# neonnnnn/nimfm

Measured on AMD Instinct MI355X. Metric: SGD training samples/sec/epoch, higher is better.
Workload: dtype f64

## Files before the change

include/nimfm_hip.h:

```cpp
#ifndef NIMFM_HIP_H
#define NIMFM_HIP_H
#include <stdint.h>

#ifdef __cplusplus
extern "C" {
#endif

#define NFM_OK 0
#define NFM_ERR_INVALID (-1)
#define NFM_ERR_HIP (-2)
#define NFM_ERR_NOT_FITTED (-3)
#define NFM_ERR_NOMEM (-4)
#define NFM_ERR_UNSUPPORTED (-5)

typedef struct nfm_ctx nfm_ctx;
typedef struct nfm_dataset nfm_dataset;
typedef struct nfm_model nfm_model;
typedef struct nfm_opt nfm_opt;

enum { NFM_TASK_REGRESSION = 0, NFM_TASK_CLASSIFICATION = 1 };
enum { NFM_KIND_FM = 0, NFM_KIND_FFM = 1, NFM_KIND_CFM = 2  };
enum { NFM_LOWER_EXPLICIT = 0, NFM_LOWER_AUGMENT = 1, NFM_LOWER_NONE = 2 };
enum { NFM_LOSS_SQUARED = 0, NFM_LOSS_SQUARED_HINGE = 1, NFM_LOSS_LOGISTIC = 2, NFM_LOSS_HUBER = 3 };
enum { NFM_SCHED_CONSTANT = 0, NFM_SCHED_OPTIMAL = 1, NFM_SCHED_INVSCALING = 2, NFM_SCHED_PEGASOS = 3 };
// ... 57 lines not shown
enum { NFM_LAYOUT_CSR = 0, NFM_LAYOUT_CSC = 1 };
int32_t nfm_dataset_create_csc(nfm_ctx* ctx, int64_t n_samples, int64_t n_features,
                               const int64_t* indptr , const int64_t* indices ,
                               const double* data , const double* y , nfm_dataset** out);
int32_t nfm_dataset_create_csc_device(nfm_ctx* ctx, int64_t n_samples, int64_t n_features, int64_t nnz,
                                      const int64_t* indptr_dev, const int32_t* indices_dev, const double* data_dev,
                                      const double* y_dev, nfm_dataset** out);
int32_t nfm_dataset_to_csc(nfm_dataset* ds, nfm_dataset** out);
int32_t nfm_dataset_to_csr(nfm_dataset* ds, nfm_dataset** out);
int32_t nfm_dataset_layout(const nfm_dataset* ds, int32_t* layout);
int32_t nfm_dataset_get_csc(nfm_dataset* ds, int64_t* indptr , int64_t* indices , double* data );
int32_t nfm_dataset_load_user_item_lines(nfm_ctx* ctx, const char* path, int32_t short_lines, nfm_dataset** out);
int32_t nfm_dataset_parse_user_item_lines(nfm_ctx* ctx, const char* text, int64_t len, int32_t short_lines, nfm_dataset** out);
int32_t nfm_dataset_shape(const nfm_dataset* ds, int64_t* n_samples, int64_t* n_features,
                          int64_t* nnz, int64_t* n_fields);
int32_t nfm_dataset_ingest_stats(const nfm_dataset* ds, int64_t* bytes, double* upload_ms,
                                 double* parse_ms);
int32_t nfm_dataset_get_targets(nfm_dataset* ds, double* y );
int32_t nfm_dataset_get_csr(nfm_dataset* ds, int64_t* indptr , int64_t* indices ,
                            double* data , int64_t* fields );
int32_t nfm_dataset_set_targets(nfm_dataset* ds, const double* y);
int32_t nfm_dataset_destroy(nfm_dataset* ds);

typedef struct nfm_model_cfg {
  int32_t kind;
  int32_t task;
  int32_t degree;
  int32_t n_components;
  int32_t fit_lower;
  int32_t fit_intercept;
// ... 129 lines not shown
```

nimfm_amd/_capi.py:

```python
import atexit
import ctypes as C
import os
import subprocess

_HERE = os.path.dirname(os.path.abspath(__file__))
LIB_PATH = os.environ.get("NIMFM_HIP_LIB") or os.path.join(_HERE, "lib", "libnimfm_hip.so")
CSRC = os.path.join(_HERE, "csrc")

NFM_OK = 0
ERR_INVALID, ERR_HIP, ERR_NOT_FITTED, ERR_NOMEM, ERR_UNSUPPORTED = -1, -2, -3, -4, -5

TASK = {"regression": 0, "r": 0, "classification": 1, "c": 1}
KIND_FM, KIND_FFM, KIND_CFM = 0, 1, 2
LOWER = {"explicit": 0, "augment": 1, "none": 2}
LOSS = {"squared": 0, "squared_hinge": 1, "logistic": 2, "huber": 3}
SCHED = {"constant": 0, "optimal": 1, "invscaling": 2, "pegasos": 3}
MODE = {"sequential": 0, "minibatch": 1}
REG = {"l1": 0, "l21": 1, "squaredl12": 2, "squaredl21": 3, "omegati": 4, "omegacs": 5}
NORM = {"l1": 0, "l2": 1, "linfty": 2}
LAYOUT = {"csr": 0, "csc": 1}

SYMBOLS = [
    "nfm_last_error", "nfm_version", "nfm_device_count",
    "nfm_ctx_create", "nfm_ctx_destroy", "nfm_ctx_synchronize",
# ... 11 lines not shown
    "nfm_dp_unique_id", "nfm_dp_create", "nfm_dp_create_local", "nfm_dp_info", "nfm_dp_destroy", "nfm_opt_set_dp", "nfm_opt_set_dp_combine", "nfm_opt_set_touch_cap", "nfm_opt_set_ada_cross",
    "nfm_opt_set_shuffle", "nfm_opt_get_perm", "nfm_opt_announce_perm",
    "nfm_stream_open", "nfm_stream_shape", "nfm_stream_load_rows", "nfm_stream_prefetch_rows", "nfm_stream_close",
    "nfm_cd_create", "nfm_cd_begin_fit", "nfm_cd_schedule", "nfm_pcd_create", "nfm_pbcd_create",
    "nfm_pgd_create", "nfm_pgd_begin_fit", "nfm_pgd_last_iter",
    "nfm_katyusha_create", "nfm_katyusha_begin_fit", "nfm_katyusha_snapshot",
    "nfm_cfm_create", "nfm_cfm_set_params", "nfm_cfm_get_params",
    "nfm_hazan_create", "nfm_hazan_begin_fit", "nfm_hazan_iter", "nfm_rng_rand_uniform",
    "nfm_gcd_create", "nfm_gcd_begin_fit", "nfm_gcd_outer_begin", "nfm_gcd_inner", "nfm_gcd_outer_end",
    "nfm_psgd_create", "nfm_psgd_begin_fit", "nfm_psgd_finalize",
    "nfm_dataset_select_rows", "nfm_dataset_slice_rows", "nfm_dataset_vstack", "nfm_dataset_hstack", "nfm_dataset_normalize",
    "nfm_dataset_load_user_item", "nfm_dataset_parse_user_item", "nfm_rng_shuffle_forward",
    "nfm_dataset_dump_svmlight", "nfm_dataset_dump_ffm", "nfm_dataset_format_text", "nfm_dump_stats", "nfm_format_f64",
    "nfm_dataset_create_csc", "nfm_dataset_create_csc_device", "nfm_dataset_to_csc", "nfm_dataset_to_csr", "nfm_dataset_layout", "nfm_dataset_get_csc",
    "nfm_dataset_load_user_item_lines", "nfm_dataset_parse_user_item_lines",
]


class ModelCfg(C.Structure):
    _fields_ = [("kind", C.c_int32), ("task", C.c_int32), ("degree", C.c_int32), ("n_components", C.c_int32),
                ("fit_lower", C.c_int32), ("fit_intercept", C.c_int32), ("fit_linear", C.c_int32),
                ("reserved", C.c_int32), ("n_features", C.c_int64), ("n_fields", C.c_int64)]


class SGDCfg(C.Structure):
    _fields_ = [("eta0", C.c_double), ("alpha0", C.c_double), ("alpha", C.c_double), ("beta", C.c_double),
                ("power", C.c_double), ("loss_param", C.c_double), ("loss", C.c_int32), ("scheduling", C.c_int32),
                ("mode", C.c_int32), ("reserved", C.c_int32), ("batch", C.c_int64)]


# ... 156 lines not shown
        "nfm_dataset_hstack": [vp, i64, pp],
        "nfm_dataset_normalize": [vp, i32, i32, pp],
        "nfm_dataset_load_user_item": [vp, C.c_char_p, pp],
        "nfm_dataset_parse_user_item": [vp, C.c_char_p, i64, pp],
        "nfm_rng_shuffle_forward": [vp, vp, i64],
        "nfm_dataset_dump_svmlight": [vp, C.c_char_p, vp, i32, i64],
        "nfm_dataset_dump_ffm": [vp, C.c_char_p, vp, i32, i64],
        "nfm_dataset_format_text": [vp, vp, i32, i64, vp, i64, C.POINTER(i64)],
        "nfm_dump_stats": [C.POINTER(i64), C.POINTER(i64), C.POINTER(dbl), C.POINTER(dbl), C.POINTER(dbl)],
        "nfm_format_f64": [vp, vp, i64, i64, vp, i64, C.POINTER(i64)],
        "nfm_dataset_create_csc": [vp, i64, i64, vp, vp, vp, vp, pp],
        "nfm_dataset_create_csc_device": [vp, i64, i64, i64, vp, vp, vp, vp, pp],
        "nfm_dataset_to_csc": [vp, pp],
        "nfm_dataset_to_csr": [vp, pp],
        "nfm_dataset_layout": [vp, C.POINTER(i32)],
        "nfm_dataset_get_csc": [vp, vp, vp, vp],
        "nfm_dataset_load_user_item_lines": [vp, C.c_char_p, i32, pp],
        "nfm_dataset_parse_user_item_lines": [vp, C.c_char_p, i64, i32, pp],
    }
    for name, args in sig.items():
        fn = getattr(L, name)
        fn.argtypes = args
        fn.restype = C.c_int32
    _lib = L
    return L


def check(rc):
    if rc == NFM_OK:
        return
# ... 7 lines not shown
```

nimfm_amd/csrc/api.hip:

```cpp
#include <fcntl.h>
#include <math.h>
#include <string.h>
#include <unistd.h>

#include <algorithm>
#include <atomic>
#include <condition_variable>
#include <map>
#include <mutex>
#include <memory>
#include <string>
#include <thread>
#include <vector>

#include "cd.h"
#include "cfm.h"
#include "dataset_csc.h"
#include "dataset_ops.h"
#include "dataset_text.h"
#include "gcd.h"
#include "psgd_seq.h"
#include "dp.h"
#include "ingest.h"
#include "mb.h"
#include "katyusha.h"
#include "pgd.h"

using namespace nfm;

struct nfm_dataset {
  nfm_ctx* ctx = nullptr;
  CsrView v{};
  DevBuf indptr, indices, data, fields, y;
  bool has_y = false;
  int max_row = 0;
  int64_t repeats = 0, repeat_row = -1;
  int64_t ingest_bytes = 0;
  double ingest_upload_ms = 0.0, ingest_parse_ms = 0.0;
  uint64_t uid = 0, serial = 0;
  uint64_t y_gen = 0;
  CscIndex csc;
  int layout = NFM_LAYOUT_CSR;
  DevBuf c_indptr, c_indices, c_data;
  CsrView cv{};
};
static int refuse_csc(const nfm_dataset* ds, const char* what) {
  NFM_CHECK(ds->layout != NFM_LAYOUT_CSC, NFM_ERR_UNSUPPORTED,
            "%s takes a row-major dataset, not a CSCDataset: convert it with toCSRDataset (nfm_dataset_to_csr)", what);
  return NFM_OK;
}
static uint64_t next_dataset_uid() {
// ... 347 lines not shown
    NFM_HIP_CHECK(hipStreamSynchronize(st));
  }
  if (y) {
    NFM_TRY(ds->y.alloc(sizeof(double) * n));
    NFM_HIP_CHECK(hipMemcpyAsync(ds->y.p, y, sizeof(double) * n, hipMemcpyHostToDevice, st));
    ds->has_y = true;
  }
  NFM_HIP_CHECK(hipStreamSynchronize(st));
  ds->v.indptr = ds->indptr.as<int64_t>();
  ds->v.indices = ds->indices.as<int32_t>();
  ds->v.data = ds->data.as<double>();
  ds->v.fields = fields ? ds->fields.as<int32_t>() : nullptr;
  ds->v.y = ds->has_y ? ds->y.as<double>() : nullptr;
  ds->v.n = n; ds->v.d = d; ds->v.nnz = nnz; ds->v.n_fields = fields ? (int32_t)n_fields : 0;
  ds->v.max_row = max_row;
  NFM_TRY(check_rows_distinct(ctx, ds->v, &ds->repeats, &ds->repeat_row));
  *out = ds.release();
  return NFM_OK;
}

int32_t nfm_dataset_create_csr_device(nfm_ctx* ctx, int64_t n, int64_t d, int64_t nnz, const int64_t* indptr_dev,
                                      const int32_t* indices_dev, const double* data_dev, const int32_t* fields_dev,
                                      int64_t n_fields, const double* y_dev, nfm_dataset** out) {
  NFM_CHECK(ctx && out && indptr_dev, NFM_ERR_INVALID, "null argument");
  NFM_CHECK(n >= 0 && d >= 0 && nnz >= 0 && d < (int64_t)2147483647 - 64, NFM_ERR_INVALID, "bad shape");
  NFM_CHECK(nnz == 0 || (indices_dev && data_dev), NFM_ERR_INVALID, "null indices/data");
  NFM_TRY(use_device(ctx));
  std::vector<int64_t> ip((size_t)n + 1);
  NFM_HIP_CHECK(hipMemcpyAsync(ip.data(), indptr_dev, sizeof(int64_t) * (n + 1), hipMemcpyDeviceToHost, ctx->stream));
  NFM_HIP_CHECK(hipStreamSynchronize(ctx->stream));
  NFM_CHECK(ip[0] == 0 && ip[n] == nnz, NFM_ERR_INVALID, "indptr[0] != 0 or indptr[n] != nnz");
  int64_t mr = 0;
  for (int64_t i = 0; i < n; ++i) {
    NFM_CHECK(ip[i + 1] >= ip[i], NFM_ERR_INVALID, "indptr not non-decreasing at row %lld", (long long)i);
    mr = std::max(mr, ip[i + 1] - ip[i]);
  }
  std::unique_ptr<nfm_dataset> ds(new nfm_dataset());
  ds->ctx = ctx;
  ds->uid = next_dataset_uid();
  ds->max_row = (int)mr;
  ds->has_y = y_dev != nullptr;
  ds->v.indptr = indptr_dev; ds->v.indices = indices_dev; ds->v.data = data_dev; ds->v.fields = fields_dev;
  ds->v.y = y_dev; ds->v.n = n; ds->v.d = d; ds->v.nnz = nnz; ds->v.n_fields = fields_dev ? (int32_t)n_fields : 0;
  ds->v.max_row = (int32_t)mr;
  NFM_TRY(check_rows_distinct(ctx, ds->v, &ds->repeats, &ds->repeat_row));
  *out = ds.release();
  return NFM_OK;
}

int32_t nfm_dataset_set_targets(nfm_dataset* ds, const double* y) {
  NFM_CHECK(ds && y, NFM_ERR_INVALID, "null argument");
  NFM_TRY(use_device(ds->ctx));
  NFM_TRY(ds->y.ensure(sizeof(double) * ds->v.n));
  NFM_HIP_CHECK(hipMemcpyAsync(ds->y.p, y, sizeof(double) * ds->v.n, hipMemcpyHostToDevice, ds->ctx->stream));
  NFM_HIP_CHECK(hipStreamSynchronize(ds->ctx->stream));
  ds->has_y = true;
  ds->y_gen++;
  if (ds->v.y != ds->y.as<double>()) ds->serial++;
  ds->v.y = ds->y.as<double>();
  return NFM_OK;
// ... 18 lines not shown
  if (with_fields) ds->fields.take(r.fields);
  ds->has_y = true;
  ds->v.indptr = ds->indptr.as<int64_t>();
  ds->v.indices = ds->indices.as<int32_t>();
  ds->v.data = ds->data.as<double>();
  ds->v.fields = with_fields ? ds->fields.as<int32_t>() : nullptr;
  ds->v.y = ds->y.as<double>();
  ds->v.n = r.n;
  ds->v.d = std::max<int64_t>(r.d, n_features);
  ds->v.nnz = r.nnz;
  ds->v.n_fields = with_fields ? (int32_t)std::max<int64_t>(r.n_fields, n_fields) : 0;
  ds->v.max_row = r.max_row;
  ds->ingest_bytes = r.bytes;
  ds->ingest_upload_ms = r.upload_ms;
  ds->ingest_parse_ms = r.parse_ms;
  NFM_TRY(check_rows_distinct(ctx, ds->v, &ds->repeats, &ds->repeat_row));
  *out = ds.release();
  return NFM_OK;
}

int32_t nfm_dataset_load_svmlight(nfm_ctx* ctx, const char* path, int64_t n_features, nfm_dataset** out) {
  NFM_CHECK(ctx && path && out, NFM_ERR_INVALID, "null argument");
  NFM_TRY(use_device(ctx));
  IngestResult r;
  NFM_TRY(ingest_text(ctx, path, nullptr, 0, false, &r));
  return dataset_from_ingest(ctx, r, false, n_features, 0, out);
}

int32_t nfm_dataset_load_ffm(nfm_ctx* ctx, const char* path, int64_t n_features, int64_t n_fields, nfm_dataset** out) {
  NFM_CHECK(ctx && path && out, NFM_ERR_INVALID, "null argument");
  NFM_TRY(use_device(ctx));
// ... 28 lines not shown
  ds->indices.take(r.indices);
  ds->data.take(r.data);
  if (r.has_fields) ds->fields.take(r.fields);
  if (r.has_y) ds->y.take(r.y);
  ds->has_y = r.has_y;
  ds->v.indptr = ds->indptr.as<int64_t>();
  ds->v.indices = ds->indices.as<int32_t>();
  ds->v.data = ds->data.as<double>();
  ds->v.fields = r.has_fields ? ds->fields.as<int32_t>() : nullptr;
  ds->v.y = r.has_y ? ds->y.as<double>() : nullptr;
  ds->v.n = r.n; ds->v.d = r.d; ds->v.nnz = r.nnz; ds->v.n_fields = r.has_fields ? (int32_t)r.n_fields : 0;
  ds->v.max_row = r.max_row;
  ds->ingest_bytes = r.bytes;
  ds->ingest_upload_ms = r.upload_ms;
  ds->ingest_parse_ms = r.parse_ms;
  NFM_TRY(check_rows_distinct(ctx, ds->v, &ds->repeats, &ds->repeat_row));
  *out = ds.release();
  return NFM_OK;
}

static int check_indices_row(const nfm_dataset* ds, int64_t m, int64_t lo, int64_t hi) {
  NFM_CHECK(m >= 1, NFM_ERR_INVALID, "Invalid slice: nSamples < 1.");
  NFM_CHECK(hi < ds->v.n, NFM_ERR_INVALID, "max(indicesRow) %lld >= %lld.", (long long)hi, (long long)ds->v.n);
  NFM_CHECK(lo >= 0, NFM_ERR_INVALID, "min(indicesRow) %lld < 0.", (long long)lo);
  return NFM_OK;
}

int32_t nfm_dataset_select_rows(nfm_dataset* ds, const int64_t* rows, int64_t m, nfm_dataset** out) {
  NFM_CHECK(ds && out && (rows || m < 1), NFM_ERR_INVALID, "null argument");
  NFM_TRY(refuse_csc(ds, "X[indices] (Accessing row vectors by openarray is not supported for CSCMatrix)"));
  int64_t lo = 0, hi = 0;
// ... 130 lines not shown
  NFM_TRY(use_device(ctx));
  DsParts r;
  if (ds->layout == NFM_LAYOUT_CSC) {
    NFM_TRY(dsop_transpose(ctx, ds->cv, &r));
    if (ds->has_y) NFM_TRY(copy_targets(ctx, ds->v.y, ds->v.n, &r.y));
    r.has_y = ds->has_y;
  } else {
    NFM_TRY(dsop_select_rows(ctx, ds->v, nullptr, 0, ds->v.n, &r));
  }
  return dataset_from_parts(ctx, r, out);
}

int32_t nfm_dataset_layout(const nfm_dataset* ds, int32_t* layout) {
  NFM_CHECK(ds && layout, NFM_ERR_INVALID, "null argument");
  *layout = ds->layout;
  return NFM_OK;
}

int32_t nfm_dataset_get_csc(nfm_dataset* ds, int64_t* indptr, int64_t* indices, double* data) {
  NFM_CHECK(ds, NFM_ERR_INVALID, "null dataset");
  NFM_CHECK(ds->layout == NFM_LAYOUT_CSC, NFM_ERR_INVALID, "the dataset is row-major: nfm_dataset_get_csr reads it (or convert it with nfm_dataset_to_csc)");
  NFM_TRY(use_device(ds->ctx));
  hipStream_t st = ds->ctx->stream;
  const int64_t d = ds->cv.n, nnz = ds->cv.nnz;
  if (indptr) NFM_HIP_CHECK(hipMemcpyAsync(indptr, ds->cv.indptr, sizeof(int64_t) * (d + 1), hipMemcpyDeviceToHost, st));
  if (data && nnz) NFM_HIP_CHECK(hipMemcpyAsync(data, ds->cv.data, sizeof(double) * nnz, hipMemcpyDeviceToHost, st));
  if (indices && nnz) {
    std::vector<int32_t> tmp((size_t)nnz);
    NFM_HIP_CHECK(hipMemcpyAsync(tmp.data(), ds->cv.indices, sizeof(int32_t) * nnz, hipMemcpyDeviceToHost, st));
    NFM_HIP_CHECK(hipStreamSynchronize(st));
// ... 1627 lines not shown
static int mb_epoch(nfm_opt* o, nfm_model* m, nfm_dataset* ds, const int64_t* perm, int64_t begin, int64_t end, double* out2) {
  nfm_ctx* ctx = m->ctx;
  hipStream_t st = ctx->stream;
  const ModelView M = m->view();
  const MbCall c = mb_call(o, m, ds, perm, begin, end);
  NFM_TRY(mb_obtain_plan(c));
  const int64_t* announced = o->ahead.take_offer(begin, end);
  if (c.dev_shuffle || o->kind == OPT_PSGD) announced = nullptr;
  DpEpoch de;
  if (o->dp) NFM_TRY(dp_epoch_open(o, m, M, &de));
  DpHooksGuard dp_guard{o};
  static const bool prefetch_on = !(getenv("NFM_PLAN_PREFETCH") && atoi(getenv("NFM_PLAN_PREFETCH")) == 0);
  const bool prefetch = (c.dev_shuffle || announced) && !ctx->timing.enabled && prefetch_on;
  if (prefetch) NFM_TRY(o->ahead.ensure_resources());
  double* out2_dst = prefetch ? o->ahead.out2_pinned : out2;
  const int rc_epoch = m->cfg.kind == NFM_KIND_FM
                           ? mb_fm_epoch(ctx, o->kind, ds->v, M, o->o, *o->plan, o->W, o->it, out2_dst, (ds->uid << 20) ^ ds->serial, prefetch)
                           : mb_ffm_epoch(ctx, o->kind, ds->v, M, o->o, *o->plan, o->W, o->it, out2_dst, prefetch);
  if (prefetch) {
    const int rc_next = rc_epoch == NFM_OK ? mb_build_ahead(c, announced) : NFM_OK;
    NFM_HIP_CHECK(hipStreamSynchronize(st));
    out2[0] = out2_dst[0];
    out2[1] = out2_dst[1];
    NFM_TRY(rc_next);
  }
  if (c.dev_shuffle) o->shuffle_epoch++;
  NFM_TRY(rc_epoch);
  if (o->dp) {
    NFM_TRY(dp_fold_pending(de));
    NFM_TRY(dp_epoch_close(o, de, out2, c.ns()));
// ... 297 lines not shown
```

nimfm_amd/csrc/mb.h:

```cpp
#pragma once
#include <functional>
#include <vector>

#include "opt_views.h"
#include "plan.h"

namespace nfm {

struct MbWork {
  DevBuf Abuf;
  DevBuf rec;
  DevBuf dLbuf;
  DevBuf dLt;
  DevBuf Wt;
  DevBuf partsA;
  DevBuf partsB;
  DevBuf Dtab;
  DevBuf Stab;
  DevBuf Ftab;
  DevBuf out_acc;
  DevBuf contrib;
  DevBuf itbuf;
  DevBuf hpart;
  DevBuf prox;
  bool use_graph = true;
  void* graph_exec = nullptr;
  uint64_t graph_plan_serial = 0;
  uint64_t graph_data_serial = 0;
  int graph_opt = -1;
// ... 25 lines not shown
```

nimfm_amd/csrc/mb_fm.hip:

```cpp
#include "mb_fm_kernels.h"

namespace nfm {

#define NFM_DECL(LL) \
  int mb_fm_run_L##LL(nfm_ctx* ctx, int opt_kind, bool gen, const CsrView& X, const ModelView& M, const OptView& O, const Plan& P, MbWork& W, int TA);
NFM_DECL(1) NFM_DECL(2) NFM_DECL(4) NFM_DECL(8) NFM_DECL(16) NFM_DECL(32) NFM_DECL(64)
#undef NFM_DECL


__global__ void k_schedule(OptView O, int fit_linear, int fit_intercept, const int64_t* __restrict__ bat_pos,
                           const double* __restrict__ it0p, double* __restrict__ Dtab ,
                           double* __restrict__ Ftab ) {
  __shared__ double red[3][kBlock];
  const double it0 = *it0p;
  const int b = blockIdx.x;
  const int64_t p0 = bat_pos[b], p1 = bat_pos[b + 1];
  double dP = 1.0, dw = 1.0, d0 = 1.0;
  for (int64_t p = p0 + threadIdx.x; p < p1; p += kBlock) {
    const double it = it0 + (double)p;
    dP *= 1 - dev::get_eta(O.sched, O.eta0, O.power, O.beta, it) * O.beta;
    if (fit_linear) dw *= 1 - dev::get_eta(O.sched, O.eta0, O.power, O.alpha, it) * O.alpha;
    if (fit_intercept) d0 *= 1 - dev::get_eta(O.sched, O.eta0, O.power, O.alpha0, it) * O.alpha0;
  }
  red[0][threadIdx.x] = dP;
// ... 119 lines not shown
      on[u] = false;
      j[u] = 0;
      if (pib[u] < len) {
        const int64_t pos = p0 + pib[u];
        const int64_t i = perm ? perm[pos] : begin + pos;
        const int64_t q0 = X.indptr[i];
        if (q < X.indptr[i + 1] - q0) {
          j[u] = X.indices[q0 + q];
          on[u] = j[u] >= j_lo && j[u] < j_hi;
        }
      }
    }
#pragma unroll
    for (int u = 0; u < U; ++u)
      if (on[u]) Wt[(size_t)pib[u] * cap + q] = w[j[u]];
  }
}

void MbWork::drop_graph() {
  if (graph_exec) (void)hipGraphExecDestroy(reinterpret_cast<hipGraphExec_t>(graph_exec));
  graph_exec = nullptr;
  for (void* e : seg_execs)
    if (e) (void)hipGraphExecDestroy(reinterpret_cast<hipGraphExec_t>(e));
  seg_execs.clear();
  seg_cut.clear();
  seg_key = -1;
}
int MbWork::seg_cut_here(nfm_ctx* ctx, int64_t b) {
  hipGraph_t graph = nullptr;
  NFM_HIP_CHECK(hipStreamEndCapture(ctx->stream, &graph));
// ... 133 lines not shown
```

nimfm_amd/csrc/mb_fm_kernels.h:

```cpp
#pragma once
#include "fm_device.h"
#include "mb.h"

namespace nfm {

#ifndef NFM_WAVE_STAGE2
#define NFM_WAVE_STAGE2 1
#endif
#ifndef NFM_COL_MINW
#define NFM_COL_MINW 1
#endif
#ifndef NFM_COL_D3
#define NFM_COL_D3 1
#endif
#ifndef NFM_REG_NTSEL
#define NFM_REG_NTSEL 0
#endif
#ifndef NFM_ADA2_MINW
#define NFM_ADA2_MINW 2
#endif

struct SampleRec {
  double dL, etaP, etaw, yhat;
};
// ... 2149 lines not shown
  __syncthreads();
  if (threadIdx.x == 0) {
    double v = 0.0;
    for (int w_ = 0; w_ < kWavesPerBlock; ++w_) v += red[0][w_];
    a.parts[a.nS + blockIdx.x] = v;
  }
  if (!closer) return;
  col_closer<OPT>(a, red);
}

__global__ void k_epoch_close(const double* __restrict__ parts, int n, double* __restrict__ out_acc);

__global__ void k_stage_dl(const int32_t* __restrict__ tpos, const double* __restrict__ dLbuf, double* __restrict__ dLt, int64_t nt);
__global__ void k_stage_w(CsrView X, const int64_t* __restrict__ perm, int64_t begin, int64_t p0, int len, int cap,
                          const double* __restrict__ w, double* __restrict__ Wt, int64_t slice_w, int wg_per_slice);
constexpr size_t kStageSliceBytes = (size_t)2 << 20;

template <int L, int SPLIT, int OPT, bool GEN>
static void launch_row(hipStream_t st, const RowArgs& ra, int mode, int n_cu, int* n_blocks) {
  const bool sing = ra.single != nullptr;
  constexpr int SPW = kWave / (L * SPLIT);
  const int nA = (ra.len + kWavesPerBlock * SPW - 1) / (kWavesPerBlock * SPW);
  *n_blocks = nA;
  constexpr bool CAN_HOLD = held_entries<L, SPLIT>() > 0;
  constexpr bool CAN_REG = CAN_HOLD && !GEN && OPT == OPT_SGD && L * SPLIT == kWave;
  if (CAN_REG && mode == 2 && ra.nt)
    hipLaunchKernelGGL((k_row_phase<L, SPLIT, OPT, GEN, (CAN_REG ? 4 : 0), false>), dim3(nA), dim3(kBlock), 0, st, ra);
  else if (CAN_REG && mode == 2)
    hipLaunchKernelGGL((k_row_phase<L, SPLIT, OPT, GEN, (CAN_REG ? 2 : 0), false>), dim3(nA), dim3(kBlock), 0, st, ra);
  else if (CAN_HOLD && mode == 3)
// ... 22 lines not shown
  const double* it0p = W.itbuf.as<double>();
  const double avg_row = X.n > 0 ? (double)X.nnz / (double)X.n + M.n_aug : 0.0;
  const size_t partsB_half = W.partsB.bytes / sizeof(double) / 2;
  const char* tu_env = getenv("NFM_TU");
  const int tu = tu_env ? atoi(tu_env) : 2;
  const bool have_singles = !GEN && P.use_singles;
  const char* long_env = getenv("NFM_COL_LONG");
  const int col_long_knob = long_env ? (atoi(long_env) != 0 ? 1 : 0) : -1;
  const char* compact_env = getenv("NFM_COL_LONG_COMPACT");
  const bool col_long_compact = !(compact_env && atoi(compact_env) == 0) &&
                                (OPT != OPT_SGD || O.power == 1.0 || (O.sched != NFM_SCHED_OPTIMAL && O.sched != NFM_SCHED_INVSCALING));
  const char* sdl_env = getenv("NFM_STAGE_DL");
  const int stage_dl_knob = sdl_env ? (atoi(sdl_env) != 0 ? 1 : 0) : -1;
  const char* sw_env = getenv("NFM_STAGE_W");
  const int stage_w_knob = sw_env ? (atoi(sw_env) != 0 ? 1 : 0) : -1;
  const char* grid_env = getenv("NFM_COL_GRID");
  const int col_grid = grid_env ? atoi(grid_env) : 0;
  static const int stream_env = getenv("NFM_STREAM") ? atoi(getenv("NFM_STREAM")) : -1;
  const size_t table_bytes = sizeof(double) * (size_t)M.nb * M.da * M.Kp * (OPT == OPT_ADAGRAD ? 3 : 1);
  const bool stream_rows = stream_env >= 0 ? stream_env != 0 : (have_singles && table_bytes > ((size_t)384 << 20));
  static const bool env_kernel = getenv("NFM_SINGLES_KERNEL") && atoi(getenv("NFM_SINGLES_KERNEL")) != 0;
  const bool singles_in_row = have_singles && !env_kernel;
  const bool singles_in_col = have_singles && !singles_in_row;
  int n_prev = 0;
  const int64_t b_first = std::min(W.batch_begin, P.n_batches), b_last = W.batch_end < 0 ? P.n_batches : std::min(W.batch_end, P.n_batches);
  for (int64_t b = b_first; b < b_last; ++b) {
    const int64_t p0 = P.bat_pos[b];
    const int len = (int)(P.bat_pos[b + 1] - p0);
    const int use_stored = (OPT == OPT_PSGD || (OPT == OPT_ADAGRAD && P.first_singleton && b == 0)) ? 1 : 0;
    const double it_b = OPT == OPT_PSGD ? (double)b : (double)p0;
// ... 33 lines not shown
    const int s_row = (R >= 16 && split >= 16) ? 16 : (R >= 8 && split >= 8) ? 8 : (R >= 4 && split >= 4) ? 4 : (R >= 2 && split >= 2) ? 2 : 1;
    const int w_cap = held_capacity(L, s_row);
    const bool stage_w = OPT == OPT_SGD && !GEN && M.fit_linear && mode_for(s_row) == 1 && stage_w_knob != 0 && col_long_compact &&
                         (stage_w_knob == 1 || col_long) && W.Wt.p != nullptr &&
                         W.Wt.bytes >= sizeof(double) * (size_t)len * (size_t)w_cap;
    int nA;
    {
      RowArgs ra{X, M, O, P.has_perm ? P.perm.as<int64_t>() : nullptr, P.begin, p0, len, use_stored, TA, stream_rows ? 1 : 0, it_b, it0p,
                 OPT == OPT_SGD ? Stab + 2 * b : M.sc, OPT == OPT_SGD ? Stab + 2 * (b + 1) : M.sc,
                 singles_in_row ? P.toff.as<int64_t>() : nullptr,
                 singles_in_row ? P.single.as<uint8_t>() : nullptr, W.Abuf.as<double>(), W.rec.as<SampleRec>(),
                 W.partsA.as<PartA>(), W.dLbuf.as<double>(), stage_w ? W.Wt.as<double>() : nullptr};
      TimedLaunch tl(ctx, "row_phase");
      if (stage_w) {
        ctx->timing.acc["stage_w"].launches += 1;
        const int64_t n_slices = std::max<int64_t>(1, ((int64_t)sizeof(double) * M.d + (int64_t)kStageSliceBytes - 1) / (int64_t)kStageSliceBytes);
        const int64_t slice_w = (M.d + n_slices - 1) / n_slices;
        const int spw = kWave / w_cap;
        const int64_t n_tasks = ((int64_t)len + spw - 1) / spw;
        const int wg_per_slice = (int)std::max<int64_t>(1, std::min<int64_t>((n_tasks + kWavesPerBlock - 1) / kWavesPerBlock, (int64_t)ctx->n_cu * 8));
        hipLaunchKernelGGL(k_stage_w, dim3((unsigned)(n_slices * wg_per_slice)), dim3(kBlock), 0, st, X,
                           P.has_perm ? P.perm.as<int64_t>() : nullptr, P.begin, p0, len, w_cap, M.w, W.Wt.as<double>(), slice_w, wg_per_slice);
      }
      int s_used;
      static const bool ada2_on = !(getenv("NFM_ADA2") && atoi(getenv("NFM_ADA2")) == 0);
      if (OPT == OPT_ADAGRAD && !GEN && L == 32 && ada2_on && singles_in_row && !use_stored && X.max_row + M.n_aug <= 64) {
        nA = (len + 1) / 2;
        if (stream_rows)
          hipLaunchKernelGGL((k_row_phase_ada2<OPT_ADAGRAD, true>), dim3(nA), dim3(kBlock), 0, st, ra);
        else
          hipLaunchKernelGGL((k_row_phase_ada2<OPT_ADAGRAD, false>), dim3(nA), dim3(kBlock), 0, st, ra);
        s_used = 2;
      } else
      if (R >= 16 && split >= 16) { launch_row<L, (R >= 16 ? 16 : R), ROPT, GEN>(st, ra, mode_for(R >= 16 ? 16 : R), ctx->n_cu, &nA); s_used = R >= 16 ? 16 : R; }
      else if (R >= 8 && split >= 8) { launch_row<L, (R >= 8 ? 8 : R), ROPT, GEN>(st, ra, mode_for(R >= 8 ? 8 : R), ctx->n_cu, &nA); s_used = R >= 8 ? 8 : R; }
      else if (R >= 4 && split >= 4) { launch_row<L, (R >= 4 ? 4 : R), ROPT, GEN>(st, ra, mode_for(R >= 4 ? 4 : R), ctx->n_cu, &nA); s_used = R >= 4 ? 4 : R; }
      else if (R >= 2 && split >= 2) { launch_row<L, (R >= 2 ? 2 : R), ROPT, GEN>(st, ra, mode_for(R >= 2 ? 2 : R), ctx->n_cu, &nA); s_used = R >= 2 ? 2 : R; }
// ... 83 lines not shown
```

nimfm_amd/csrc/plan.h:

```cpp
#pragma once
#include "common.h"

namespace nfm {

struct Plan {
  uint64_t serial = 0;
  uint64_t ds_uid = 0;
  int64_t ds_nnz = -1;
  int64_t begin = 0, end = 0, batch = 0;
  int n_aug = 0;
  bool first_singleton = false, has_perm = false, use_singles = false;
  int64_t n_batches = 0, U = 0, T = 0, TM = 0, max_batch = 0, max_unique = 0;
  std::vector<int64_t> bat_pos;
  std::vector<int64_t> bat_uoff;
  std::vector<int64_t> bat_toff;
  DevBuf perm;
  DevBuf bat_pos_dev;
  DevBuf ucol;
  DevBuf uptr;
  DevBuf ucol_s;
  DevBuf ubeg_s;
  DevBuf ucnt_s;
  DevBuf tpos;
  DevBuf tx;
// ... 10 lines not shown
};

struct CscIndex {
  bool built = false, usable = false;
  bool seg_unfit = false;
  int64_t max_col = 0;
  DevBuf cptr;
  DevBuf crow;
  DevBuf cval;
  DevBuf cnz;
};

constexpr int kHeavyTouches = 128;
constexpr int kHeavySegment = 64;

int check_rows_distinct(nfm_ctx* ctx, const CsrView& X, int64_t* n_repeats, int64_t* first_row);

constexpr int kFeistelRounds = 4;
struct FeistelKey {
  uint32_t k[kFeistelRounds];
  uint32_t mask;
  int h;
  int64_t ns, begin;
};
FeistelKey feistel_key(int64_t seed, uint64_t epoch, int64_t begin, int64_t ns);

int plan_build(nfm_ctx* ctx, const CsrView& X, int n_aug, const int64_t* perm_host, int64_t begin, int64_t end,
               int64_t batch, bool first_singleton, bool want_tq, bool use_singles, bool sort_by_count, Plan* out,
               hipStream_t stream = nullptr, const int64_t* perm_dev = nullptr, CscIndex* csc = nullptr,
               const FeistelKey* perm_key = nullptr);

// ... 4 lines not shown
```

nimfm_amd/csrc/plan.hip:

```cpp
#include <hipcub/hipcub.hpp>
#include <type_traits>

#include <stdlib.h>

#include <atomic>

#include "plan.h"

namespace nfm {

void Plan::release() {
  perm.release();
  bat_pos_dev.release();
  ucol.release();
  uptr.release();
  ucol_s.release();
  ubeg_s.release();
  ucnt_s.release();
  tpos.release();
  tx.release();
  tq.release();
  toff.release();
  single.release();
  hv_u.release();
// ... 179 lines not shown
  for (int64_t r = wave0; r < n; r += nwaves) {
    const int64_t q0 = indptr[r], q1 = indptr[r + 1];
    bool row_bad = false;
    for (int64_t q = q0 + 1 + lane; q < q1; q += kWave) {
      const int32_t a = ids[q - 1], b = ids[q];
      if (SORTED ? a == b : b <= a) {
        ++bad;
        row_bad = true;
      }
    }
    if (row_bad) atomicMin(first_row, (long long)r);
  }
  if (bad) atomicAdd(count, bad);
}

int check_rows_distinct(nfm_ctx* ctx, const CsrView& X, int64_t* n_repeats, int64_t* first_row) {
  *n_repeats = 0;
  *first_row = -1;
  if (X.n == 0 || X.nnz < 2 || X.max_row < 2) return NFM_OK;
  hipStream_t st = ctx->stream;
  DevBuf stat;
  NFM_TRY(stat.alloc(16));
  long long h[2] = {0, INT64_MAX};
  auto run = [&](bool sorted, const int32_t* ids) -> int {
    h[0] = 0;
    h[1] = INT64_MAX;
    NFM_HIP_CHECK(hipMemcpyAsync(stat.p, h, sizeof(h), hipMemcpyHostToDevice, st));
    int64_t blocks = (X.n + kWavesPerBlock - 1) / kWavesPerBlock;
    if (blocks > 256 * 32) blocks = 256 * 32;
    if (sorted)
      hipLaunchKernelGGL(k_row_order<true>, dim3((unsigned)blocks), dim3(kBlock), 0, st, X.n, X.indptr, ids,
                         stat.as<unsigned long long>(), stat.as<long long>() + 1);
    else
      hipLaunchKernelGGL(k_row_order<false>, dim3((unsigned)blocks), dim3(kBlock), 0, st, X.n, X.indptr, ids,
                         stat.as<unsigned long long>(), stat.as<long long>() + 1);
    NFM_HIP_CHECK(hipGetLastError());
    NFM_HIP_CHECK(hipMemcpyAsync(h, stat.p, sizeof(h), hipMemcpyDeviceToHost, st));
    NFM_HIP_CHECK(hipStreamSynchronize(st));
    return NFM_OK;
  };
  NFM_TRY(run(false, X.indices));
  if (h[0] == 0) return NFM_OK;
  NFM_CHECK(X.nnz < (int64_t)2147483647, NFM_ERR_UNSUPPORTED, "more than 2^31-1 nnz with unsorted rows");
  DevBuf k0, k1, tmp;
  NFM_TRY(k0.alloc(sizeof(int32_t) * X.nnz));
  NFM_TRY(k1.alloc(sizeof(int32_t) * X.nnz));
  NFM_HIP_CHECK(hipMemcpyAsync(k0.p, X.indices, sizeof(int32_t) * X.nnz, hipMemcpyDeviceToDevice, st));
  hipcub::DoubleBuffer<int32_t> dk(k0.as<int32_t>(), k1.as<int32_t>());
  size_t bytes = 0;
  NFM_HIP_CHECK(hipcub::DeviceSegmentedRadixSort::SortKeys(nullptr, bytes, dk, (int)X.nnz, (int)X.n, X.indptr, X.indptr + 1, 0, 32, st));
  NFM_TRY(tmp.alloc(bytes));
  NFM_HIP_CHECK(hipcub::DeviceSegmentedRadixSort::SortKeys(tmp.p, bytes, dk, (int)X.nnz, (int)X.n, X.indptr, X.indptr + 1, 0, 32, st));
  NFM_TRY(run(true, dk.Current()));
  *n_repeats = h[0];
  *first_row = h[0] ? h[1] : -1;
  return NFM_OK;
}
// ... 1173 lines not shown
```

nimfm_amd/host.py:

```python
import ctypes as C
import os
import math
from types import SimpleNamespace

import numpy as np

from . import _capi as capi


def _vp(a):
    return None if a is None else a.ctypes.data_as(C.c_void_p)


def _f64(a):
    return np.ascontiguousarray(a, dtype=np.float64)


def _i64(a):
    return np.ascontiguousarray(a, dtype=np.int64)


class Context:

    def __init__(self, device_id=0, stream=None):
# ... 70 lines not shown

    @classmethod
    def _from_loader(cls, ctx, h):
        n, d, nnz, nf, lay = C.c_int64(), C.c_int64(), C.c_int64(), C.c_int64(), C.c_int32()
        capi.check(capi.lib().nfm_dataset_shape(h, C.byref(n), C.byref(d), C.byref(nnz), C.byref(nf)))
        capi.check(capi.lib().nfm_dataset_layout(h, C.byref(lay)))
        kind = CSCDataset if lay.value == capi.LAYOUT["csc"] else CSRDataset
        ds = kind(nSamples=n.value, nFeatures=d.value, nFields=nf.value, ctx=ctx, _handle=h)
        ds.nnz = nnz.value
        return ds

    def targets(self):
        y = np.zeros(self.nSamples)
        capi.check(capi.lib().nfm_dataset_get_targets(self.h, _vp(y)))
        return y

    def to_host(self):
        indptr = np.zeros(self.nSamples + 1, dtype=np.int64)
        indices = np.zeros(self.nnz, dtype=np.int64)
        data = np.zeros(self.nnz)
        fields = np.zeros(self.nnz, dtype=np.int64) if self.nFields else None
        capi.check(capi.lib().nfm_dataset_get_csr(self.h, _vp(indptr), _vp(indices), _vp(data), _vp(fields)))
        return indptr, indices, data, fields

    def ingest_stats(self):
        b, u, p = C.c_int64(), C.c_double(), C.c_double()
        capi.check(capi.lib().nfm_dataset_ingest_stats(self.h, C.byref(b), C.byref(u), C.byref(p)))
        return b.value, u.value, p.value

    @property
# ... 2297 lines not shown
```

Baseline: 88.13 million.

## Stage weights by column-position passes when row indices are sorted ascending

Records at dataset creation whether every row's feature indices are already ascending, and carries that flag into the minibatch workspace. When it holds, the weight-staging step launches a new kernel that splits each row's held entries into a few position ranges (passes) instead of slicing the feature space into 2MB windows. Since sorted rows give increasing indices by position, each pass should gather from a narrower band of the weight vector, aiming for better cache locality with fewer redundant scans. It adds an env knob and a new code path whose benefit depends on the index distribution.

```diff
diff --git a/include/nimfm_hip.h b/include/nimfm_hip.h
--- a/include/nimfm_hip.h
+++ b/include/nimfm_hip.h
@@ -95,6 +95,7 @@
 int32_t nfm_dataset_parse_user_item_lines(nfm_ctx* ctx, const char* text, int64_t len, int32_t short_lines, nfm_dataset** out);
 int32_t nfm_dataset_shape(const nfm_dataset* ds, int64_t* n_samples, int64_t* n_features,
                           int64_t* nnz, int64_t* n_fields);
+int32_t nfm_dataset_rows_ascend(const nfm_dataset* ds, int32_t* ascend);
 int32_t nfm_dataset_ingest_stats(const nfm_dataset* ds, int64_t* bytes, double* upload_ms,
                                  double* parse_ms);
 int32_t nfm_dataset_get_targets(nfm_dataset* ds, double* y );
diff --git a/nimfm_amd/_capi.py b/nimfm_amd/_capi.py
--- a/nimfm_amd/_capi.py
+++ b/nimfm_amd/_capi.py
@@ -49,6 +49,7 @@
     "nfm_dataset_dump_svmlight", "nfm_dataset_dump_ffm", "nfm_dataset_format_text", "nfm_dump_stats", "nfm_format_f64",
     "nfm_dataset_create_csc", "nfm_dataset_create_csc_device", "nfm_dataset_to_csc", "nfm_dataset_to_csr", "nfm_dataset_layout", "nfm_dataset_get_csc",
     "nfm_dataset_load_user_item_lines", "nfm_dataset_parse_user_item_lines",
+    "nfm_dataset_rows_ascend",
 ]
 
 
@@ -235,6 +236,7 @@
         "nfm_dataset_to_csc": [vp, pp],
         "nfm_dataset_to_csr": [vp, pp],
         "nfm_dataset_layout": [vp, C.POINTER(i32)],
+        "nfm_dataset_rows_ascend": [vp, C.POINTER(i32)],
         "nfm_dataset_get_csc": [vp, vp, vp, vp],
         "nfm_dataset_load_user_item_lines": [vp, C.c_char_p, i32, pp],
         "nfm_dataset_parse_user_item_lines": [vp, C.c_char_p, i64, i32, pp],
diff --git a/nimfm_amd/csrc/api.hip b/nimfm_amd/csrc/api.hip
--- a/nimfm_amd/csrc/api.hip
+++ b/nimfm_amd/csrc/api.hip
@@ -35,6 +35,7 @@
   bool has_y = false;
   int max_row = 0;
   int64_t repeats = 0, repeat_row = -1;
+  bool rows_ascend = true;
   int64_t ingest_bytes = 0;
   double ingest_upload_ms = 0.0, ingest_parse_ms = 0.0;
   uint64_t uid = 0, serial = 0;
@@ -412,7 +413,7 @@
   ds->v.y = ds->has_y ? ds->y.as<double>() : nullptr;
   ds->v.n = n; ds->v.d = d; ds->v.nnz = nnz; ds->v.n_fields = fields ? (int32_t)n_fields : 0;
   ds->v.max_row = max_row;
-  NFM_TRY(check_rows_distinct(ctx, ds->v, &ds->repeats, &ds->repeat_row));
+  NFM_TRY(check_rows_distinct(ctx, ds->v, &ds->repeats, &ds->repeat_row, &ds->rows_ascend));
   *out = ds.release();
   return NFM_OK;
 }
@@ -441,7 +442,7 @@
   ds->v.indptr = indptr_dev; ds->v.indices = indices_dev; ds->v.data = data_dev; ds->v.fields = fields_dev;
   ds->v.y = y_dev; ds->v.n = n; ds->v.d = d; ds->v.nnz = nnz; ds->v.n_fields = fields_dev ? (int32_t)n_fields : 0;
   ds->v.max_row = (int32_t)mr;
-  NFM_TRY(check_rows_distinct(ctx, ds->v, &ds->repeats, &ds->repeat_row));
+  NFM_TRY(check_rows_distinct(ctx, ds->v, &ds->repeats, &ds->repeat_row, &ds->rows_ascend));
   *out = ds.release();
   return NFM_OK;
 }
@@ -490,7 +491,7 @@
   ds->ingest_bytes = r.bytes;
   ds->ingest_upload_ms = r.upload_ms;
   ds->ingest_parse_ms = r.parse_ms;
-  NFM_TRY(check_rows_distinct(ctx, ds->v, &ds->repeats, &ds->repeat_row));
+  NFM_TRY(check_rows_distinct(ctx, ds->v, &ds->repeats, &ds->repeat_row, &ds->rows_ascend));
   *out = ds.release();
   return NFM_OK;
 }
@@ -549,7 +550,7 @@
   ds->ingest_bytes = r.bytes;
   ds->ingest_upload_ms = r.upload_ms;
   ds->ingest_parse_ms = r.parse_ms;
-  NFM_TRY(check_rows_distinct(ctx, ds->v, &ds->repeats, &ds->repeat_row));
+  NFM_TRY(check_rows_distinct(ctx, ds->v, &ds->repeats, &ds->repeat_row, &ds->rows_ascend));
   *out = ds.release();
   return NFM_OK;
 }
@@ -710,6 +711,12 @@
 int32_t nfm_dataset_layout(const nfm_dataset* ds, int32_t* layout) {
   NFM_CHECK(ds && layout, NFM_ERR_INVALID, "null argument");
   *layout = ds->layout;
+  return NFM_OK;
+}
+
+int32_t nfm_dataset_rows_ascend(const nfm_dataset* ds, int32_t* ascend) {
+  NFM_CHECK(ds && ascend, NFM_ERR_INVALID, "null argument");
+  *ascend = ds->rows_ascend ? 1 : 0;
   return NFM_OK;
 }
 
@@ -2367,6 +2374,7 @@
   const bool prefetch = (c.dev_shuffle || announced) && !ctx->timing.enabled && prefetch_on;
   if (prefetch) NFM_TRY(o->ahead.ensure_resources());
   double* out2_dst = prefetch ? o->ahead.out2_pinned : out2;
+  o->W.rows_ascend = ds->rows_ascend;
   const int rc_epoch = m->cfg.kind == NFM_KIND_FM
                            ? mb_fm_epoch(ctx, o->kind, ds->v, M, o->o, *o->plan, o->W, o->it, out2_dst, (ds->uid << 20) ^ ds->serial, prefetch)
                            : mb_ffm_epoch(ctx, o->kind, ds->v, M, o->o, *o->plan, o->W, o->it, out2_dst, prefetch);
diff --git a/nimfm_amd/csrc/mb.h b/nimfm_amd/csrc/mb.h
--- a/nimfm_amd/csrc/mb.h
+++ b/nimfm_amd/csrc/mb.h
@@ -13,6 +13,7 @@
   DevBuf dLbuf;
   DevBuf dLt;
   DevBuf Wt;
+  bool rows_ascend = false;
   DevBuf partsA;
   DevBuf partsB;
   DevBuf Dtab;
diff --git a/nimfm_amd/csrc/mb_fm.hip b/nimfm_amd/csrc/mb_fm.hip
--- a/nimfm_amd/csrc/mb_fm.hip
+++ b/nimfm_amd/csrc/mb_fm.hip
@@ -157,6 +157,43 @@
 #pragma unroll
     for (int u = 0; u < U; ++u)
       if (on[u]) Wt[(size_t)pib[u] * cap + q] = w[j[u]];
+  }
+}
+
+__global__ __launch_bounds__(kBlock) void k_stage_w_ranges(CsrView X, const int64_t* __restrict__ perm, int64_t begin, int64_t p0, int len,
+                                                            int cap, const double* __restrict__ w, double* __restrict__ Wt, int n_pass,
+                                                            int wg_per_pass) {
+  constexpr int U = 4;
+  const int pass = blockIdx.x / wg_per_pass, wg = blockIdx.x % wg_per_pass;
+  const int lane = threadIdx.x & (kWave - 1), wv = threadIdx.x >> 6;
+  const int W = cap / n_pass;
+  const int spw = kWave / W, sub = lane / W, q = pass * W + lane % W;
+  const int64_t n_tasks = ((int64_t)len + spw - 1) / spw;
+  for (int64_t t = ((int64_t)wg * kWavesPerBlock + wv) * U; t < n_tasks; t += (int64_t)wg_per_pass * kWavesPerBlock * U) {
+    int64_t pib[U];
+    int j[U];
+    bool on[U];
+#pragma unroll
+    for (int u = 0; u < U; ++u) {
+      pib[u] = (t + u) * spw + sub;
+      on[u] = false;
+      j[u] = 0;
+      if (pib[u] < len) {
+        const int64_t pos = p0 + pib[u];
+        const int64_t i = perm ? perm[pos] : begin + pos;
+        const int64_t q0 = X.indptr[i];
+        if (q < X.indptr[i + 1] - q0) {
+          j[u] = X.indices[q0 + q];
+          on[u] = true;
+        }
+      }
+    }
+    double v[U];
+#pragma unroll
+    for (int u = 0; u < U; ++u) v[u] = on[u] ? w[j[u]] : 0.0;
+#pragma unroll
+    for (int u = 0; u < U; ++u)
+      if (on[u]) Wt[(size_t)pib[u] * cap + q] = v[u];
   }
 }
 
diff --git a/nimfm_amd/csrc/mb_fm_kernels.h b/nimfm_amd/csrc/mb_fm_kernels.h
--- a/nimfm_amd/csrc/mb_fm_kernels.h
+++ b/nimfm_amd/csrc/mb_fm_kernels.h
@@ -2187,6 +2187,9 @@
 __global__ void k_stage_dl(const int32_t* __restrict__ tpos, const double* __restrict__ dLbuf, double* __restrict__ dLt, int64_t nt);
 __global__ void k_stage_w(CsrView X, const int64_t* __restrict__ perm, int64_t begin, int64_t p0, int len, int cap,
                           const double* __restrict__ w, double* __restrict__ Wt, int64_t slice_w, int wg_per_slice);
+__global__ void k_stage_w_ranges(CsrView X, const int64_t* __restrict__ perm, int64_t begin, int64_t p0, int len, int cap,
+                                 const double* __restrict__ w, double* __restrict__ Wt, int n_pass, int wg_per_pass);
+constexpr int kStagePasses = 4;
 constexpr size_t kStageSliceBytes = (size_t)2 << 20;
 
 template <int L, int SPLIT, int OPT, bool GEN>
@@ -2239,6 +2242,8 @@
   const int stage_dl_knob = sdl_env ? (atoi(sdl_env) != 0 ? 1 : 0) : -1;
   const char* sw_env = getenv("NFM_STAGE_W");
   const int stage_w_knob = sw_env ? (atoi(sw_env) != 0 ? 1 : 0) : -1;
+  const char* swp_env = getenv("NFM_STAGE_W_PASSES");
+  const int stage_w_passes = swp_env ? atoi(swp_env) : (W.rows_ascend ? kStagePasses : 0);
   const char* grid_env = getenv("NFM_COL_GRID");
   const int col_grid = grid_env ? atoi(grid_env) : 0;
   static const int stream_env = getenv("NFM_STREAM") ? atoi(getenv("NFM_STREAM")) : -1;
@@ -2302,13 +2307,25 @@
       TimedLaunch tl(ctx, "row_phase");
       if (stage_w) {
         ctx->timing.acc["stage_w"].launches += 1;
-        const int64_t n_slices = std::max<int64_t>(1, ((int64_t)sizeof(double) * M.d + (int64_t)kStageSliceBytes - 1) / (int64_t)kStageSliceBytes);
-        const int64_t slice_w = (M.d + n_slices - 1) / n_slices;
-        const int spw = kWave / w_cap;
-        const int64_t n_tasks = ((int64_t)len + spw - 1) / spw;
-        const int wg_per_slice = (int)std::max<int64_t>(1, std::min<int64_t>((n_tasks + kWavesPerBlock - 1) / kWavesPerBlock, (int64_t)ctx->n_cu * 8));
-        hipLaunchKernelGGL(k_stage_w, dim3((unsigned)(n_slices * wg_per_slice)), dim3(kBlock), 0, st, X,
-                           P.has_perm ? P.perm.as<int64_t>() : nullptr, P.begin, p0, len, w_cap, M.w, W.Wt.as<double>(), slice_w, wg_per_slice);
+        if (stage_w_passes != 0) {
+          NFM_CHECK(stage_w_passes > 0 && stage_w_passes <= w_cap && (stage_w_passes & (stage_w_passes - 1)) == 0, NFM_ERR_INVALID,
+                    "NFM_STAGE_W_PASSES=%d: 0 or a power of two up to the row phase's %d held entries", stage_w_passes, w_cap);
+          ctx->timing.acc["stage_w_ranges"].launches += 1;
+          const int spw = kWave / (w_cap / stage_w_passes);
+          const int64_t n_tasks = ((int64_t)len + spw - 1) / spw;
+          const int wg_per_pass = (int)std::max<int64_t>(1, std::min<int64_t>((n_tasks + kWavesPerBlock - 1) / kWavesPerBlock, (int64_t)ctx->n_cu * 8));
+          hipLaunchKernelGGL(k_stage_w_ranges, dim3((unsigned)(stage_w_passes * wg_per_pass)), dim3(kBlock), 0, st, X,
+                             P.has_perm ? P.perm.as<int64_t>() : nullptr, P.begin, p0, len, w_cap, M.w, W.Wt.as<double>(), stage_w_passes,
+                             wg_per_pass);
+        } else {
+          const int64_t n_slices = std::max<int64_t>(1, ((int64_t)sizeof(double) * M.d + (int64_t)kStageSliceBytes - 1) / (int64_t)kStageSliceBytes);
+          const int64_t slice_w = (M.d + n_slices - 1) / n_slices;
+          const int spw = kWave / w_cap;
+          const int64_t n_tasks = ((int64_t)len + spw - 1) / spw;
+          const int wg_per_slice = (int)std::max<int64_t>(1, std::min<int64_t>((n_tasks + kWavesPerBlock - 1) / kWavesPerBlock, (int64_t)ctx->n_cu * 8));
+          hipLaunchKernelGGL(k_stage_w, dim3((unsigned)(n_slices * wg_per_slice)), dim3(kBlock), 0, st, X,
+                             P.has_perm ? P.perm.as<int64_t>() : nullptr, P.begin, p0, len, w_cap, M.w, W.Wt.as<double>(), slice_w, wg_per_slice);
+        }
       }
       int s_used;
       static const bool ada2_on = !(getenv("NFM_ADA2") && atoi(getenv("NFM_ADA2")) == 0);
diff --git a/nimfm_amd/csrc/plan.h b/nimfm_amd/csrc/plan.h
--- a/nimfm_amd/csrc/plan.h
+++ b/nimfm_amd/csrc/plan.h
@@ -48,7 +48,7 @@
 constexpr int kHeavyTouches = 128;
 constexpr int kHeavySegment = 64;
 
-int check_rows_distinct(nfm_ctx* ctx, const CsrView& X, int64_t* n_repeats, int64_t* first_row);
+int check_rows_distinct(nfm_ctx* ctx, const CsrView& X, int64_t* n_repeats, int64_t* first_row, bool* rows_ascend = nullptr);
 
 constexpr int kFeistelRounds = 4;
 struct FeistelKey {
diff --git a/nimfm_amd/csrc/plan.hip b/nimfm_amd/csrc/plan.hip
--- a/nimfm_amd/csrc/plan.hip
+++ b/nimfm_amd/csrc/plan.hip
@@ -217,9 +217,10 @@
   if (bad) atomicAdd(count, bad);
 }
 
-int check_rows_distinct(nfm_ctx* ctx, const CsrView& X, int64_t* n_repeats, int64_t* first_row) {
+int check_rows_distinct(nfm_ctx* ctx, const CsrView& X, int64_t* n_repeats, int64_t* first_row, bool* rows_ascend) {
   *n_repeats = 0;
   *first_row = -1;
+  if (rows_ascend) *rows_ascend = true;
   if (X.n == 0 || X.nnz < 2 || X.max_row < 2) return NFM_OK;
   hipStream_t st = ctx->stream;
   DevBuf stat;
@@ -244,6 +245,7 @@
   };
   NFM_TRY(run(false, X.indices));
   if (h[0] == 0) return NFM_OK;
+  if (rows_ascend) *rows_ascend = false;
   NFM_CHECK(X.nnz < (int64_t)2147483647, NFM_ERR_UNSUPPORTED, "more than 2^31-1 nnz with unsorted rows");
   DevBuf k0, k1, tmp;
   NFM_TRY(k0.alloc(sizeof(int32_t) * X.nnz));
diff --git a/nimfm_amd/host.py b/nimfm_amd/host.py
--- a/nimfm_amd/host.py
+++ b/nimfm_amd/host.py
@@ -108,6 +108,11 @@
         y = np.zeros(self.nSamples)
         capi.check(capi.lib().nfm_dataset_get_targets(self.h, _vp(y)))
         return y
+
+    def rows_ascend(self):
+        a = C.c_int32()
+        capi.check(capi.lib().nfm_dataset_rows_ascend(self.h, C.byref(a)))
+        return bool(a.value)
 
     def to_host(self):
         indptr = np.zeros(self.nSamples + 1, dtype=np.int64)
```

Measured after the change: 89.82 million (median of 6 runs). +1.9%, better.
